# pinterest/rocksplicator

Hardware: NVIDIA H100
Metric: multiget_lookups_per_s (higher is better)
Workload: dtype u8

## Files before the change

rocksplicator_b200/csrc/engine.cu:

```cuda
#include <algorithm>
#include <atomic>
#include <chrono>
#include <cstddef>
#include <cstdio>
#include <cstdlib>
#include <cstring>
#include <deque>
#include <functional>
#include <map>
#include <memory>
#include <mutex>
#include <stdexcept>
#include <string>
#include <thread>
#include <unordered_map>
#include <vector>

#include "../../include/rsp_b200.h"
#include "arena.h"
#include "reader_set.h"
#include "stager.h"
#include "kernels.h"

using namespace rsp;
// ... 163 lines not shown
  mutable bool reserved = false;
};

struct ReadCombiner;
struct ApplyCombiner;
struct Compactor;

struct CudaReaderApi {
  using Stream = cudaStream_t;
  using Event = cudaEvent_t;
  static Event create() {
    cudaEvent_t ev = nullptr;
    CUDA_OK(cudaEventCreateWithFlags(&ev, cudaEventDisableTiming));
    return ev;
  }
  static void record(Event ev, Stream s) { CUDA_OK(cudaEventRecord(ev, s)); }
  static void wait(Stream on, Event ev) { CUDA_OK(cudaStreamWaitEvent(on, ev, 0)); }
  static void destroy(Event ev) { cudaEventDestroy(ev); }
};

struct rsp_engine {
  int device = 0;
  std::mutex comb_mu;
  ReadCombiner* read_comb = nullptr;
  ApplyCombiner* apply_comb = nullptr;
  std::atomic<ReadCombiner*> read_comb_ready{nullptr};
  std::atomic<ApplyCombiner*> apply_comb_ready{nullptr};
  rsp_engine_cfg cfg{};
  std::mutex mu;
  cudaStream_t st = nullptr;
  cudaStream_t cs[3] = {nullptr, nullptr, nullptr};
  cudaEvent_t cs_done[3] = {nullptr, nullptr, nullptr};
  Arena arena;
  ShardDev* d_shards = nullptr;
  ShardFast* d_fast = nullptr;
  std::vector<rsp_shard*> slots;
  std::unordered_map<std::string, rsp_shard*> by_name;
  PinBuf pin_in, pin_out, pin_up, pin_totals;
  DevBuf dev_tick, dev_q, dev_pending, dev_up;
  cudaEvent_t pending_ev = nullptr;
  bool pending_ev_recorded = false;
  cudaStream_t pending_last_stream = nullptr;
  cudaEvent_t up_ev = nullptr;
  bool up_ev_recorded = false;
  std::vector<u32> gid_scratch;
  std::vector<u8> seen_scratch;
  ReaderSet<CudaReaderApi> readers;
  cudaEvent_t mut_ev = nullptr;
  bool mut_recorded = false;
  size_t stage_threads = 1;
  ShardFast* d_fast_runs = nullptr;
  u32* d_mt_filter = nullptr;
  std::atomic<u32> n_multirun{0};
  std::atomic<u32> n_string_append{0};
  struct Compactor* compactor = nullptr;
  u32 mg_parity = 0;
  size_t pending_cap = 0;
  struct {
    bool fast = false, host = false;
    u32 parity = 0;
    size_t n_chunks = 0, chunk = 0;
  } last_mg;
  cudaEvent_t ev0 = nullptr, ev1 = nullptr;
  std::map<std::string, float> last_ms;
  std::atomic<u64> launches{0};
  ScanView* d_snap_views = nullptr;
  std::vector<rsp_snapshot*> snap_slots;
};

static void set_err(rsp_shard* s, const std::string& m) {
  std::lock_guard<std::mutex> g(s->err_mu);
  s->last_error = m;
}

static void wait_readers(rsp_engine* e) { e->readers.wait(e->st); }
static void note_mutation(rsp_engine* e) {
  CUDA_OK(cudaEventRecord(e->mut_ev, e->st));
  e->mut_recorded = true;
}
static void reader_begin(rsp_engine* e, cudaStream_t s) {
  if (s != e->st && e->mut_recorded) CUDA_OK(cudaStreamWaitEvent(s, e->mut_ev, 0));
}
static void reader_end(rsp_engine* e, cudaStream_t s) {
  if (s == e->st) return;
  e->readers.note(s);
}

static void describe_shard(rsp_engine* e, rsp_shard* s, ShardFast* f_out, ShardFast* fr) {
  s->h.n_runs = (u32)s->runs.size();
  for (u32 i = 0; i < RSP_MAX_RUNS; i++) {
    if (i < s->runs.size()) s->h.runs[i] = s->runs[i]->dev();
    else memset(&s->h.runs[i], 0, sizeof(RunDev));
  }
  auto describe = [](const Run& r, ShardFast* f) {
    f->run0_heap = (u64)r.heap; f->run0_hslots = (u64)r.hslots; f->n_buckets = r.n_buckets;
    f->meta = r.ord_bits | (std::min<u32>(r.uniform_units, 255u) << FAST_META_UNITS_SHIFT);
  };
  ShardFast f;
  memset(&f, 0, sizeof(f));
  if (!s->runs.empty()) describe(*s->runs[0], &f);
  memset(fr, 0, sizeof(ShardFast) * RSP_MAX_RUNS);
  for (size_t i = 0; i < s->runs.size() && i < RSP_MAX_RUNS; i++) describe(*s->runs[i], &fr[i]);
  const bool multi_now = s->runs.size() > 1;
  if (multi_now != s->counted_multirun) {
    if (multi_now) e->n_multirun++; else e->n_multirun--;
    s->counted_multirun = multi_now;
// ... 263 lines not shown
      while (at < s->runs.size() && s->runs[at].get() != h.srcs.front().get()) at++;
      bool intact = at + h.n_merged <= s->runs.size();
      for (size_t k = 0; intact && k < h.n_merged; k++) intact = s->runs[at + k].get() == h.srcs[k].get();
      s->merging = false;
      s->bg_first_pinned = nullptr;
      if (!intact) { h.s = nullptr; continue; }
    }
    u64 read_b = 0;
    if (h.has_mem) read_b += (u64)s->h.mt_tail * 16;
    for (auto& r : h.srcs) read_b += r->bytes();
    s->stats.compaction_bytes_read += read_b;
    s->stats.compaction_bytes_written += plan->outs[i]->bytes();
    if (h.has_mem) s->stats.flushes++;
    if (h.has_mem && h.generic_sort) s->stats.flush_comparison_sorts++;
    size_t at = 0;
    if (h.n_merged) {
      while (at < s->runs.size() && s->runs[at].get() != h.srcs.front().get()) at++;
      s->stats.compactions++;
      s->runs.erase(s->runs.begin() + at, s->runs.begin() + at + h.n_merged);
    }
    if (plan->outs[i]->n_ent) s->runs.insert(s->runs.begin() + at, plan->outs[i]);
    if (h.has_mem) {
      s->h.mt_tail = 0;
      s->h.mt_count = 0;
    }
    stage_upload(e, s, mode == COMPACT_MERGE, h.has_mem, &up);
  }
  commit_uploads(e, &up);
  note_mutation(e);
  CUDA_OK(cudaStreamSynchronize(e->st));
  e->last_ms["compact"] = plan->ms;
  e->last_ms["compact_total"] += plan->ms;
  for (u32 i = 0; i < nj; i++) {
    rsp_shard* s = plan->jh[i].s;
    if (s && s->runs.size() >= e->cfg.l0_compaction_trigger && !s->merging) bg_request(e, s);
  }
}

static void compact_shards(rsp_engine* e, const std::vector<rsp_shard*>& shards, bool force_full) {
  CompactPlan plan;
  const CompactMode mode = force_full ? COMPACT_FULL : COMPACT_FLUSH;
  plan_jobs(e, shards, mode, &plan);
  if (plan.jobs.empty()) return;
  wait_readers(e);
  try {
    run_jobs(e, &plan, e->st, e->ev0, e->ev1, &e->pin_totals);
  } catch (...) {
    cudaStreamSynchronize(e->st);
    release_work(e, &plan);
    throw;
  }
  install_jobs(e, &plan, mode);
  release_work(e, &plan);
}

static std::shared_ptr<Run> snapshot_memtable(rsp_engine* e, rsp_shard* s) {
  CompactPlan plan;
  plan_jobs(e, {s}, COMPACT_SNAPSHOT, &plan);
  if (plan.jobs.empty()) return nullptr;
  try {
    run_jobs(e, &plan, e->st, e->ev0, e->ev1, &e->pin_totals);
  } catch (...) {
    cudaStreamSynchronize(e->st);
    release_work(e, &plan);
    throw;
  }
  release_work(e, &plan);
  s->stats.compaction_bytes_read += (u64)s->h.mt_tail * 16;
  return plan.outs[0]->n_ent ? plan.outs[0] : nullptr;
}

static void view_of(const rsp_shard* s, const std::vector<std::shared_ptr<Run>>& pinned, ScanView* v) {
  memset(v, 0, sizeof(*v));
  v->n_runs = (u32)pinned.size();
  v->merge_op = s->opts.merge_op;
  v->merge_delim = s->h.merge_delim;
  for (u32 i = 0; i < v->n_runs; i++) v->runs[i] = pinned[i]->dev();
}

static void pin_view(rsp_engine* e, rsp_shard* s, std::vector<std::shared_ptr<Run>>* pinned, ScanView* v) {
  pinned->clear();
  if (s->h.mt_count) {
    wait_readers(e);
    if (auto snap = snapshot_memtable(e, s)) pinned->push_back(snap);
  }
  pinned->insert(pinned->end(), s->runs.begin(), s->runs.end());
  if (pinned->size() > RSP_MAX_RUNS) {
    pinned->clear();
    compact_shards(e, {s}, false);
    *pinned = s->runs;
  }
  view_of(s, *pinned, v);
}

struct Compactor {
  rsp_engine* e = nullptr;
  std::mutex mu;
  std::condition_variable cv;
  std::vector<rsp_shard*> pending;
  bool stop = false, busy = false;
  cudaStream_t stream = nullptr;
  cudaEvent_t ev0 = nullptr, ev1 = nullptr;
  PinBuf pin_totals;
  std::thread th;
  void loop();
};
// ... 261 lines not shown
    f.chunks = (const ChunkDesc*)(dev + dev_b_base); f.n_chunks = (u32)chunks.size(); f.pad = 0;
    f.chain = (u64*)(dev + dev_b_base + align_up(chunks.size() * sizeof(ChunkDesc), 256));
    f.group_done = (u32*)((u8*)f.chain + chunks.size() * 32);
    if (!chunks.empty())
      CUDA_OK(cudaMemcpyAsync(dev + dev_b_base, chunks.data(), chunks.size() * sizeof(ChunkDesc), cudaMemcpyHostToDevice, e->st));
  }
  if (own_dev) CUDA_OK(cudaStreamSynchronize(e->st));
  return RSP_OK;
}

static void unreserve(const rsp_staged* sg) {
  if (!sg->reserved) return;
  for (size_t g = 0; g < sg->group_shard.size(); g++) {
    rsp_shard* s = sg->group_shard[g];
    s->inflight_units -= std::min<u64>(s->inflight_units, sg->need_units[g]);
    s->inflight_ents -= std::min<u64>(s->inflight_ents, sg->need_ents[g]);
  }
  sg->reserved = false;
}

static inline bool ticks_in_flight(const rsp_shard* s) { return s->inflight_units != 0 || s->inflight_ents != 0; }

static int reserve_for(rsp_engine* e, const rsp_staged* sg) {
  bool did_work = false;
  unreserve(sg);
  auto fits = [](const rsp_shard* s, u64 nu, u64 ne) {
    const u64 tail = (u64)s->h.mt_tail + s->inflight_units, cnt = (u64)s->h.mt_count + s->inflight_ents;
    return tail + nu <= s->h.mt_heap_cap && cnt + ne <= s->h.mt_ent_cap && (cnt + ne) * 2 <= (u64)s->h.mt_slot_mask + 1;
  };
  std::vector<rsp_shard*> to_flush;
  for (size_t g = 0; g < sg->group_shard.size(); g++) {
    rsp_shard* s = sg->group_shard[g];
    if (fits(s, sg->need_units[g], sg->need_ents[g])) continue;
    if (s->inflight_units || s->inflight_ents) return -1;
    if (s->h.mt_count) to_flush.push_back(s);
  }
  if (!to_flush.empty()) { compact_shards(e, to_flush, false); did_work = true; }
  UploadBatch up;
  try {
    for (size_t g = 0; g < sg->group_shard.size(); g++) {
      rsp_shard* s = sg->group_shard[g];
      const u64 nu = sg->need_units[g], ne = sg->need_ents[g];
      if (!fits(s, nu, ne)) {
        alloc_memtable(e, s, nu + nu / 2, ne + ne / 2);
        stage_upload(e, s, false, true, &up);
        did_work = true;
      }
    }
  } catch (...) {
    commit_uploads(e, &up);
    throw;
  }
  commit_uploads(e, &up);
  for (size_t g = 0; g < sg->group_shard.size(); g++) {
    sg->group_shard[g]->inflight_units += sg->need_units[g];
    sg->group_shard[g]->inflight_ents += sg->need_ents[g];
  }
  sg->reserved = true;
  return did_work ? 1 : 0;
}

static void tick_launch(rsp_engine* e, rsp_staged* sg, cudaStream_t st) {
  if (sg->fused) {
    launch_tick_fused(sg->ftick, e->d_shards, e->d_fast, e->d_mt_filter, st);
    CUDA_OK(cudaGetLastError());
    e->launches += 1;
    return;
  }
  launch_decode(sg->tick, st);
  launch_sequence(sg->tick, e->d_shards, e->d_fast, st);
  launch_insert(sg->tick, e->d_shards, e->d_mt_filter, st);
  launch_publish(sg->tick, e->d_shards, st);
  CUDA_OK(cudaGetLastError());
  e->launches += 4;
}

static int tick_results(rsp_engine* e, rsp_staged* sg, cudaStream_t st, int32_t* st_out) {
  u8* pout = (u8*)e->pin_out.get(sg->res_bytes);
  CUDA_OK(cudaMemcpyAsync(pout, sg->tick.gres, sg->res_bytes, cudaMemcpyDeviceToHost, st));
  CUDA_OK(cudaStreamSynchronize(st));
  float ms = 0;
  if (cudaEventElapsedTime(&ms, e->ev0, e->ev1) == cudaSuccess) e->last_ms["apply"] = ms;
  unreserve(sg);
  const size_t ng = sg->group_shard.size();
  const GroupRes* gr = (const GroupRes*)pout;
  const u32* bs = (const u32*)(pout + ng * sizeof(GroupRes));
  int worst = RSP_OK;
  for (size_t g = 0; g < ng; g++) {
    rsp_shard* s = sg->group_shard[g];
    s->h.last_seq = gr[g].last_seq;
    s->h.pub_seq = gr[g].last_seq;
    s->h.mt_tail = gr[g].tail;
    s->h.mt_count = gr[g].count;
    s->h.latch = gr[g].latch;
    s->latch = gr[g].latch;
    s->last_seq.store(gr[g].last_seq, std::memory_order_release);
  }
  bool any_bad = false;
  for (size_t p = 0; p < sg->n; p++) {
    const u32 code = bs[p] >> 8;
    if (st_out) st_out[sg->identity_order ? p : sg->order[p]] = (int32_t)code;
    any_bad |= code != 0;
  }
  if (any_bad) {
    for (size_t g = 0; g < ng; g++) {
      for (u32 p = sg->group_first[g]; p < sg->group_first[g + 1]; p++) {
// ... 205 lines not shown
    size_t n_ops = recs.size();
    if (recs.back().type != kTypeMerge) {
      n_ops--;
      if (recs.back().type == kTypeValue) { has = true; cur = recs.back().v; }
    }
    if (n_ops == 0) {
      if (!has) return RSP_NOT_FOUND;
      *value = cur;
      return RSP_OK;
    }
    const std::string k((const char*)key, klen);
    for (size_t i = n_ops; i-- > 0;) {
      std::string nv;
      if (!host_merge_one(s, k, has, cur, recs[i].v, &nv)) {
        set_err(s, kMsgText[MSG_MERGE_FAILED]);
        return RSP_CORRUPTION;
      }
      cur.swap(nv);
      has = true;
    }
    *value = cur;
    return RSP_OK;
  }
}

static void pending_order(rsp_engine* e, cudaStream_t stream) {
  if (e->pending_ev_recorded && e->pending_last_stream != stream) CUDA_OK(cudaStreamWaitEvent(stream, e->pending_ev, 0));
}
static void pending_mark(rsp_engine* e, cudaStream_t stream) {
  CUDA_OK(cudaEventRecord(e->pending_ev, stream));
  e->pending_ev_recorded = true;
  e->pending_last_stream = stream;
}
static void set_pending(rsp_engine* e, GetArgs& a, size_t n, cudaStream_t stream) {
  pending_order(e, stream);
  if ((n + 8) * 4 > e->pending_cap) {
    if (e->pending_ev_recorded) CUDA_OK(cudaEventSynchronize(e->pending_ev));
    e->pending_cap = std::max<size_t>((n + 8) * 4, e->pending_cap * 2);
    u32* p = (u32*)e->dev_pending.get(e->pending_cap);
    CUDA_OK(cudaMemsetAsync(p, 0, 16, stream));
    e->mg_parity = 0;
  }
  a.n_special = (u32*)e->dev_pending.p;
  a.n_pending = (u32*)e->dev_pending.p + 2;
  a.pending = a.n_pending + 2;
  a.parity = e->mg_parity;
  e->mg_parity ^= 1u;
}

static bool cat_reads(const rsp_engine* e) { return e->n_string_append.load() != 0; }

static void set_engine_args(rsp_engine* e, GetArgs& a) {
  a.shards = e->d_shards; a.fast = e->d_fast; a.max_shards = e->cfg.max_shards;
  a.multirun = e->n_multirun.load() ? 1u : 0u;
}

static inline bool plain_status(int32_t st) { return st == RSP_OK || st == RSP_NOT_FOUND || st == RSP_INCOMPLETE; }

struct LookupRef {
  rsp_shard* s;
  const uint8_t* key;
  size_t klen;
  const ScanView* d_view;
};
template <class Ref>
static void finish_special(rsp_engine* e, size_t n, Ref ref, uint8_t* vals, size_t val_stride, uint32_t* vlen, int32_t* st) {
  for (size_t i = 0; i < n; i++) {
    if (plain_status(st[i])) continue;
    const LookupRef r = ref(i);
    if (st[i] == ST_NEED_HOST_MERGE) {
      std::string v;
      const int rc = host_fold_get(e, r.s, r.key, r.klen, &v, r.d_view);
      st[i] = rc;
      vlen[i] = 0;
      if (rc == RSP_OK) {
        vlen[i] = (u32)v.size();
        if (v.size() > val_stride) st[i] = RSP_INCOMPLETE;
        else memcpy(vals + i * val_stride, v.data(), v.size());
      }
    } else {
      const u32 msg = vlen[i];
      if (r.s) set_err(r.s, msg < MSG_COUNT ? kMsgText[msg] : "error");
      vlen[i] = 0;
    }
  }
}

static int multi_get_locked(rsp_engine* e, size_t n, const uint32_t* shard_ix, const uint8_t* keys, const uint64_t* koff,
                            uint32_t klen_fixed, uint8_t* vals, size_t val_stride, uint32_t* vlen, int32_t* st) {
  if (n == 0) return RSP_OK;
  const size_t key_bytes = klen_fixed ? n * klen_fixed : (size_t)koff[n];
  QLayout L;
  const size_t o_six = L.add(n * 4), o_koff = L.add(klen_fixed ? 0 : (n + 1) * 8), o_keys = L.add(key_bytes + 16);
  const size_t o_vlen = L.add(n * 4), o_st = L.add(n * 4), o_vals = L.add(n * val_stride + 256);
  u8* d = (u8*)e->dev_q.get(L.size);
  const size_t CH = 1u << 18;
  const bool piped = klen_fixed && n >= 2 * CH;
  const size_t n_chunks = piped ? (n + CH - 1) / CH : 1;
  const size_t scratch_u32 = 4 + 2 * n_chunks + n + 16;
  if (e->pending_ev_recorded) {
    CUDA_OK(cudaEventSynchronize(e->pending_ev));
    e->pending_ev_recorded = false;
  }
  if (scratch_u32 * 4 > e->pending_cap) {
    e->pending_cap = std::max(scratch_u32 * 4, e->pending_cap * 2);
    e->dev_pending.get(e->pending_cap);
  }
// ... 1775 lines not shown
```

rocksplicator_b200/csrc/k_read.cu:

```cuda
#include <algorithm>
#include <cstddef>
#include <type_traits>

#include "kernels.h"

namespace rsp {

__device__ __forceinline__ u64 ldcg64(const void* p) { return __ldcg(reinterpret_cast<const unsigned long long*>(p)); }
__device__ __forceinline__ u32 ldcg32(const void* p) { return __ldcg(reinterpret_cast<const u32*>(p)); }

struct CatState {
  u8* out;
  u64 cap;
  u32 len;
  u32 delim;
  u32 gmask;
};
struct NoCat {};

__device__ __noinline__ void cat_put_reversed(u8* out, u64 cap, u64 at, const u8* src, u32 n, u32 delim, u32 gmask) {
  const u32 lanes = __popc(gmask), lane = __popc(gmask & ((1u << (threadIdx.x & 31u)) - 1u));
  for (u32 b = lane; b < n; b += lanes) {
    const u64 p = at + n - 1u - b;
    if (p < cap) out[p] = __ldcg(src + b);
// ... 249 lines not shown
    if ((u64)vlen > a.val_stride) {
      st = 7;
    } else {
      u8* dst = a.vals + (u64)q * a.val_stride;
      if (acc.imm) {
        if (lane == 0) {
#pragma unroll
          for (u32 b = 0; b < 8; b++) dst[b] = (u8)(acc.res_imm >> (8u * b));
        }
      } else if (!acc.in_place(dst)) {
        group_copy_out(dst, acc.res_ptr, vlen, lane, MG_LANES);
      }
    }
  } else if (st != 1 && st != ST_NEED_HOST_MERGE) {
    vlen = msg;
  }
  if (lane == 0) {
    a.st[q] = st;
    a.vlen[q] = vlen;
    if (st != 0 && st != 1 && st != 7 && a.n_special) atomicAdd(a.n_special, 1u);
  }
}

template <bool CAT>
__device__ __noinline__ void lookup_generic(const GetArgs& a, u32 q, u32 lane, u32 gmask, u32 gbase) {
  const u32 six = __ldg(a.shard_ix + q);
  if (six >= a.max_shards || !a.shards[six].live) return answer_invalid(a, q, lane);
  const ShardDev* sd = a.shards + six;
  u32 klen;
  const u8* kp = lookup_key(a, q, klen);
  Acc<CAT> acc;
  acc.init(sd->merge_op, sd->merge_delim);
  acc.set_out(a.vals + (u64)q * a.val_stride, a.val_stride, gmask);
  walk_shard<MG_LANES>(sd, kp, klen, lane, gmask, gbase, acc);
  answer(a, q, lane, acc);
}

template <bool CAT>
__global__ void __launch_bounds__(256) k_multi_get(GetArgs a) {
  const u32 q = (blockIdx.x * blockDim.x + threadIdx.x) / MG_LANES;
  const u32 lane = threadIdx.x & (MG_LANES - 1);
  const u32 gbase = (threadIdx.x & 31u) & ~(MG_LANES - 1u);
  const u32 gmask = ((1u << MG_LANES) - 1u) << gbase;
  if (q >= a.n) return;
  lookup_generic<CAT>(a, q, lane, gmask, gbase);
}

static_assert(offsetof(ShardDev, mt_slot_mask) == 24 && offsetof(ShardDev, pub_seq) == 56, "ShardDev units 0-3");
static_assert(sizeof(ShardFast) == 32, "ShardFast");

constexpr u32 FL = 2;
constexpr u32 MG16_THREADS = 64;
constexpr u32 MG16_MIN_BLOCKS = 20;

__device__ __forceinline__ u64 pol_evict_last() {
  u64 p;
#ifdef RSP_EMUL
  p = 0;
#else
  asm("createpolicy.fractional.L2::evict_last.b64 %0, 1.0;" : "=l"(p));
#endif
  return p;
}
__device__ __forceinline__ uint4 ldg_pol(const uint4* p, u64 pol) {
  uint4 v;
#ifdef RSP_EMUL
  (void)pol;
  v = *p;
#else
  asm("ld.global.nc.L2::cache_hint.v4.u32 {%0,%1,%2,%3}, [%4], %5;"
      : "=r"(v.x), "=r"(v.y), "=r"(v.z), "=r"(v.w) : "l"(p), "l"(pol));
#endif
  return v;
}

template <bool CG>
__device__ __forceinline__ uint4 ld_entry_unit(const uint4* p) {
  if (CG) return __ldcg(p);
  return __ldg(p);
}
template <bool CG, bool BIG>
__device__ __forceinline__ u32 fast_entry(const u8* ent, u32 U, u32 KU, const uint4& kq, u64 snap, u8* dst,
                                          u64 val_stride, u32 lane, u32& vlen_out) {
  const uint4* ep = reinterpret_cast<const uint4*>(ent);
  const uint4 hd = ld_entry_unit<CG>(ep);
  const uint4 ek = ld_entry_unit<CG>(ep + KU);
  const u32 fv = KU + 1;
  uint4 v0 = make_uint4(0, 0, 0, 0), v1 = v0, v2 = v0;
  if (!CG) {
    if (fv + lane < U) v0 = ld_entry_unit<CG>(ep + fv + lane);
    if (fv + lane + 2 < U) v1 = ld_entry_unit<CG>(ep + fv + lane + 2);
    if (fv + lane + 4 < U) v2 = ld_entry_unit<CG>(ep + fv + lane + 4);
  }
  if (ek.x != kq.x || ek.y != kq.y || ek.z != kq.z || ek.w != kq.w || hd.z != 16) return 1;
  const u64 seq = (((u64)hd.y << 32) | hd.x) >> 8;
  const u32 vu = (hd.w + 15u) >> 4;
  if ((hd.x & 0xffu) != kTypeValue || seq > snap || (!CG && fv + vu > U) || (u64)vu * 16u > val_stride || (!BIG && vu > 6)) return 2;
  uint4* out = reinterpret_cast<uint4*>(dst);
  if (CG) {
    for (u32 u = lane; u < vu; u += FL) out[u] = ld_entry_unit<CG>(ep + fv + u);
  } else {
    if (lane < vu) out[lane] = v0;
    if (lane + 2 < vu) out[lane + 2] = v1;
    if (lane + 4 < vu) out[lane + 4] = v2;
    if (BIG)
      for (u32 u = lane + 6; u < vu; u += FL) out[u] = ld_entry_unit<CG>(ep + fv + u);
  }
  vlen_out = hd.w;
  return 0;
}

template <bool BIG>
__device__ __forceinline__ u32 probe_one_run(const uint4& g0, const uint4& g1, const uint4& kq, u64 h, u8* dst, u64 val_stride,
                                             u32 lane, u32 pmask, u32 pbase, u32& vlen) {
  const u8* heap = reinterpret_cast<const u8*>(((u64)g0.y << 32) | g0.x);
  const u32 n_buckets = g1.x, ord_bits = g1.y & 0xffu, U = (g1.y >> FAST_META_UNITS_SHIFT) & 0xffu;
  if (U == 0 || U >= 255) return 2;
  const uint4* hs = reinterpret_cast<const uint4*>(((u64)g0.w << 32) | g0.z);
  u32 bucket = (u32)(((u64)(u32)h * n_buckets) >> 32);
  const u32 tag = (u32)(h >> 32) >> ord_bits;
  u32 m8 = 0, e8 = 1, probe = 0;
  uint4 sv = make_uint4(0, 0, 0, 0);
#pragma unroll 1
  for (;;) {
    if (!m8) {
      if (probe && e8) return 4;
      if (probe == n_buckets) return 4;
      if (probe) bucket = bucket + 1 == n_buckets ? 0 : bucket + 1;
      probe++;
      sv = ldg_pol(hs + (u64)bucket * 2u + lane, pol_evict_last());
      const u32 m = ((sv.x && (sv.x >> ord_bits) == tag) ? 1u : 0u) | ((sv.y && (sv.y >> ord_bits) == tag) ? 2u : 0u) |
                    ((sv.z && (sv.z >> ord_bits) == tag) ? 4u : 0u) | ((sv.w && (sv.w >> ord_bits) == tag) ? 8u : 0u);
      const u32 e = (sv.x == 0 || sv.y == 0 || sv.z == 0 || sv.w == 0) ? 1u : 0u;
      const u32 mine = m | (e << 4);
      const u32 other = __shfl_xor_sync(pmask, mine, 1);
      m8 = lane ? ((other & 15u) | ((mine & 15u) << 4)) : ((mine & 15u) | ((other & 15u) << 4));
      e8 = (mine | other) >> 4;
      if (!m8) continue;
    }
    const u32 p = __ffs(m8) - 1;
    m8 &= m8 - 1;
    const u32 pick = (p & 2u) ? ((p & 1u) ? sv.w : sv.z) : ((p & 1u) ? sv.y : sv.x);
    const u32 val = __shfl_sync(pmask, pick, pbase + (p >> 2));
    const u32 r = fast_entry<false, BIG>(heap + (u64)((val & ((1u << ord_bits) - 1u)) - 1u) * U * 16u, U, 1, kq, ~0ull, dst,
                                         val_stride, lane, vlen);
    if (r == 0) return 0;
    if (r == 2) return 2;
  }
}

template <bool BIG, bool MULTI>
__device__ __forceinline__ void multi_get16(GetArgs a) {
  const u32 q = (blockIdx.x * blockDim.x + threadIdx.x) / FL;
  const u32 lane = threadIdx.x & (FL - 1);
  const u32 pbase = (threadIdx.x & 31u) & ~1u;
  const u32 pmask = 3u << pbase;
  if (q >= a.n) return;
  u32 six = __ldg(a.shard_ix + q);
  const bool bad_shard = six >= a.max_shards;
  if (bad_shard) six = 0;
  const uint4 kq = __ldg(reinterpret_cast<const uint4*>(a.keys) + q);
  const uint4 f0 = __ldg(reinterpret_cast<const uint4*>(a.fast + six));
  const uint4 f1 = __ldg(reinterpret_cast<const uint4*>(a.fast + six) + 1);
  const u32 n_runs = (f1.y >> FAST_META_RUNS_SHIFT) & 0xffu;
  const u64 k0 = ((u64)kq.y << 32) | kq.x, k1 = ((u64)kq.w << 32) | kq.z;
  const u64 h = hash_final(hash_step(hash_step(hash_init(16), k0), k1));
  u8* dst = a.vals + (u64)q * a.val_stride;
  u32 state = 3;
  u32 vlen = 0;
  if ((!MULTI && n_runs > 1) || ((a.val_stride | reinterpret_cast<uintptr_t>(a.vals)) & 15u) || bad_shard || !(f1.y & FAST_META_LIVE)) state = 2;
  bool in_mem = false;
  if (state == 3 && f1.z ) {
    const u32 fb = mt_filter_bit(h);
    const u32 fw = __ldcg(reinterpret_cast<const u32*>(a.fast + (size_t)a.max_shards * (1u + RSP_MAX_RUNS)) + (size_t)six * MT_FILTER_WORDS + (fb >> 5));
    in_mem = (fw >> (fb & 31u)) & 1u;
  }
  if (in_mem) {
    const uint4* dp = reinterpret_cast<const uint4*>(a.shards + six);
    const uint4 d0 = __ldcg(dp), d1 = __ldcg(dp + 1), d3 = __ldcg(dp + 3);
    const u8* heap = reinterpret_cast<const u8*>(((u64)d0.y << 32) | d0.x);
    const u64* sp = reinterpret_cast<const u64*>(((u64)d0.w << 32) | d0.z);
    const u32 mask = d1.z;
    const u64 snap = ((u64)d3.w << 32) | d3.z;
    const u32 tag = hash_tag32(h);
    u32 cand = 0, info = 0;
#pragma unroll
    for (u32 i = 0; i < 4; i++) {
      const u64 sv = ldcg64(sp + (((u32)h + 4u * lane + i) & mask));
      if (sv == 0) { if (!(info >> 8)) info |= (4u * lane + i + 1u) << 8; }
      else if ((u32)(sv >> 32) == tag && !(info >> 8)) { if (!cand) cand = (u32)sv; info++; }
    }
    const u32 o_cand = __shfl_xor_sync(pmask, cand, 1), o_info = __shfl_xor_sync(pmask, info, 1);
    const u32 lo_info = lane ? o_info : info, hi_info = lane ? info : o_info;
    const u32 lo_cand = lane ? o_cand : cand, hi_cand = lane ? cand : o_cand;
    const bool lo_empty = (lo_info >> 8) != 0;
    const u32 n_match = (lo_info & 0xffu) + (lo_empty ? 0u : (hi_info & 0xffu));
    const bool any_empty = lo_empty || (hi_info >> 8) != 0;
    if (n_match == 1) {
      const u32 c = (lo_info & 0xffu) ? lo_cand : hi_cand;
      const u32 r = fast_entry<true, BIG>(heap + (u64)(c - 1u) * 16u, 7, 2, kq, snap, dst, a.val_stride, lane, vlen);
      state = r == 0 ? 0 : 2;
    } else if (n_match > 1 || !any_empty) {
      state = 2;
    }
  }
  if (state == 3) {
    state = 4;
    for (u32 r = 0; r < n_runs; r++) {
      uint4 g0 = f0, g1 = f1;
      if (MULTI && r) {
        const uint4* fr = reinterpret_cast<const uint4*>(a.fast + a.max_shards) + ((u64)six * RSP_MAX_RUNS + r) * 2u;
        g0 = __ldg(fr);
        g1 = __ldg(fr + 1);
      }
      const u32 rs = probe_one_run<BIG>(g0, g1, kq, h, dst, a.val_stride, lane, pmask, pbase, vlen);
      if (rs != 4 || !MULTI) { state = rs; break; }
    }
  }
  if (lane == 0) {
    if (state == 2) {
      a.pending[atomicAdd(a.n_pending + a.parity, 1u)] = q;
    } else {
      a.st[q] = state == 0 ? 0 : 1;
      a.vlen[q] = vlen;
    }
  }
}

template <bool BIG>
__global__ void __launch_bounds__(MG16_THREADS, MG16_MIN_BLOCKS) k_multi_get16(GetArgs a) { multi_get16<BIG, false>(a); }
template <bool BIG>
__global__ void __launch_bounds__(MG16_THREADS, MG16_MIN_BLOCKS) k_multi_get16m(GetArgs a) { multi_get16<BIG, true>(a); }

template <bool CAT>
__global__ void __launch_bounds__(256) k_multi_get_pending(GetArgs a) {
  const u32 lane = threadIdx.x & (MG_LANES - 1);
  const u32 gbase = (threadIdx.x & 31u) & ~(MG_LANES - 1u);
  const u32 gmask = ((1u << MG_LANES) - 1u) << gbase;
  const u32 n = __ldcg(a.n_pending + a.parity);
  const u32 groups = gridDim.x * (blockDim.x / MG_LANES);
  for (u32 i = (blockIdx.x * blockDim.x + threadIdx.x) / MG_LANES; i < n; i += groups)
    lookup_generic<CAT>(a, __ldcg(a.pending + i), lane, gmask, gbase);
}

bool launch_multi_get(const GetArgs& a, bool cat, cudaStream_t s) {
  if (!a.n) return false;
  const u32 per_block = 256 / MG_LANES;
  const u32 grid = (a.n + per_block - 1) / per_block;
  if (a.klen_fixed == 16 && (reinterpret_cast<uintptr_t>(a.keys) & 15u) == 0 && a.pending && a.fast) {
    cudaMemsetAsync(a.n_pending + a.parity, 0, 4, s);
    const u32 g16 = (a.n + MG16_THREADS / FL - 1) / (MG16_THREADS / FL);
    const bool multi = a.multirun != 0;
    if (a.val_stride > 96) {
      if (multi) k_multi_get16m<true><<<g16, MG16_THREADS, 0, s>>>(a); else k_multi_get16<true><<<g16, MG16_THREADS, 0, s>>>(a);
    } else {
      if (multi) k_multi_get16m<false><<<g16, MG16_THREADS, 0, s>>>(a); else k_multi_get16<false><<<g16, MG16_THREADS, 0, s>>>(a);
    }
    if (cat) k_multi_get_pending<true><<<std::min<u32>(grid, DEVICE_SMS), 256, 0, s>>>(a);
    else k_multi_get_pending<false><<<std::min<u32>(grid, DEVICE_SMS), 256, 0, s>>>(a);
    return true;
  }
  if (cat) k_multi_get<true><<<grid, 256, 0, s>>>(a);
  else k_multi_get<false><<<grid, 256, 0, s>>>(a);
  return false;
}

struct DumpVisitor {
  u8* out;
  u64 cap;
  u32 used, n_rec;
  bool done;
  __device__ bool visit(u32 type, const u8* vptr, u32 vlen) {
    const u32 rec = 8u + ((vlen + 3u) & ~3u);
    if ((u64)used + rec <= cap) {
      *reinterpret_cast<u32*>(out + used) = type;
      *reinterpret_cast<u32*>(out + used + 4) = vlen;
      for (u32 b = 0; b < vlen; b++) out[used + 8 + b] = __ldcg(vptr + b);
      n_rec++;
    }
    used += rec;
    if (type != kTypeMerge) done = true;
    return done;
  }
};

__global__ void k_get_versions(VersionsArgs a) {
  const u32 q = blockIdx.x * blockDim.x + threadIdx.x;
  if (q >= a.n) return;
  const u32 lane_in_warp = threadIdx.x & 31u;
  const ShardDev* sd = a.views ? nullptr : a.shards + a.shard_ix[q];
  const u64 o = a.koff[q];
  const u32 klen = (u32)(a.koff[q + 1] - o);
  DumpVisitor v{a.out + (u64)q * a.out_stride, a.out_stride, 0, 0, false};
  if (a.views) {
    const ScanView& vw = a.views[q];
    const u64 h = hash_key(a.keys + o, klen);
    walk_runs<1>(vw.runs, vw.n_runs, a.keys + o, klen, h, 0, 1u << lane_in_warp, lane_in_warp, v);
  } else {
    walk_shard<1>(sd, a.keys + o, klen, 0, 1u << lane_in_warp, lane_in_warp, v);
  }
  a.n_rec[q] = v.n_rec;
  a.need[q] = v.used;
}

void launch_get_versions(const VersionsArgs& a, cudaStream_t s) {
  if (!a.n) return;
  k_get_versions<<<(a.n + 63) / 64, 64, 0, s>>>(a);
}

template <bool CAT>
// ... 414 lines not shown
```

rocksplicator_b200/csrc/kernels.h:

```cpp
#pragma once
#include "format.cuh"

namespace rsp {

constexpr u32 DEVICE_SMS = 132;

struct BatchDesc {
  u32 shard_ix;
  u32 boff;
  u32 len;
  u32 op_base;
  u32 op_cap;
  u32 group;
  u32 pad0, pad1;
};
struct GroupDesc {
  u32 shard_ix;
  u32 first_batch;
  u32 n_batches;
  u32 pad;
};
struct BatchRes {
  u32 status;
  u32 n_ops;
// ... 38 lines not shown
  u32 n_batches;
  u32 index_in_group;
  u32 shard_ix;
  u32 group_chunks;
  u32 pad0, pad1;
};
constexpr u32 FUSED_CHUNK_BATCHES = 128;
constexpr u32 FUSED_STAGE_BYTES = 16384;
struct FusedTick {
  const u8* blob;
  const u64* off;
  const u32* len;
  const u64* ts;
  const GroupDesc* groups;
  u32* bstat;
  GroupRes* gres;
  u32 n_groups;
  u32 n_batches;
  u32 max_group;
  u32 max_len;
  const ChunkDesc* chunks;
  u64* chain;
  u32* group_done;
  u32 n_chunks;
  u32 pad;
};
inline bool fused_small_shape(u32 max_group, u32 max_len) { return max_group <= 64 && max_len <= 4096; }
constexpr u32 FUSED_MAX_BATCH_BYTES = 16384;
void launch_tick_fused(const FusedTick& t, ShardDev* shards, ShardFast* fast, u32* mt_filter, cudaStream_t s);
void launch_decode(const TickDev& t, cudaStream_t s);
void launch_sequence(const TickDev& t, ShardDev* shards, ShardFast* fast, cudaStream_t s);
void launch_insert(const TickDev& t, ShardDev* shards, u32* mt_filter, cudaStream_t s);
void launch_publish(const TickDev& t, ShardDev* shards, cudaStream_t s);

struct GetArgs {
  const ShardDev* shards;
  const ShardFast* fast;
  const u32* shard_ix;
  const u8* keys;
  const u64* koff;
  u32 klen_fixed;
  u8* vals;
  u64 val_stride;
  u32* vlen;
  i32* st;
  u32 n;
  u32* pending;
  u32* n_pending;
  u32 parity;
  u32* n_special;
  u32 max_shards;
  u32 multirun;
};
static_assert(sizeof(GetArgs) == 128, "GetArgs layout is part of k_multi_get16's measured code generation");
bool launch_multi_get(const GetArgs& a, bool cat, cudaStream_t s);

struct ScanView;
struct VersionsArgs {
  const ShardDev* shards;
  const ScanView* views;
  const u32* shard_ix;
  const u8* keys;
  const u64* koff;
  u8* out;
  u64 out_stride;
  u32* n_rec;
  u32* need;
  u32 n;
};
void launch_get_versions(const VersionsArgs& a, cudaStream_t s);

struct ScanView {
  RunDev runs[RSP_MAX_RUNS];
  u32 n_runs;
  u32 merge_op;
  u32 live;
  u32 merge_delim;
};

struct GetAtArgs {
  const ScanView* views;
  const u32* slot;
  const u8* keys;
  const u64* koff;
  u8* vals;
  u64 val_stride;
  u32* vlen;
  i32* st;
  u32* n_special;
  u32 n_views;
  u32 klen_fixed;
  u32 n;
};
void launch_multi_get_at(const GetAtArgs& a, bool cat, cudaStream_t s);
constexpr u32 SCAN_VLEN_HOST_FOLD = 0xffffffffu;
constexpr u32 SCAN_VLEN_MERGE_FAILED = 0xfffffffeu;
constexpr i32 SCAN_ST_TRUNCATED = 1 << 30;
struct ScanArgs {
  const ShardDev* shards;
  const ScanView* views;
  const u32* shard_ix;
  const u8* keys;
  const u64* koff;
  u32 klen_fixed;
  u32 flags;
  u32 max_entries;
// ... 71 lines not shown
```

Measured before the change: 9.175 billion.

## Prefetch memtable filter word and run home buckets early in 16-byte multiget

Adds a host-tracked memtable-live flag and new kernel variants that issue the memtable filter load and the first hash-bucket loads for the first one or two runs early, before the memtable probe finishes, so their latencies overlap instead of forming a dependent chain. Second-run metadata and its prefetched bucket are parked in shared memory to limit register pressure. The memtable path speculatively loads value units bounded by the heap capacity. Launch bounds are relaxed for the new variants, which trades occupancy for more in-flight loads and adds code complexity.

```diff
diff --git a/rocksplicator_b200/csrc/engine.cu b/rocksplicator_b200/csrc/engine.cu
--- a/rocksplicator_b200/csrc/engine.cu
+++ b/rocksplicator_b200/csrc/engine.cu
@@ -239,6 +239,7 @@
   ShardFast* d_fast_runs = nullptr;
   u32* d_mt_filter = nullptr;
   std::atomic<u32> n_multirun{0};
+  std::atomic<u32> mt_live{0};
   std::atomic<u32> n_string_append{0};
   struct Compactor* compactor = nullptr;
   u32 mg_parity = 0;
@@ -608,6 +609,10 @@
   }
   install_jobs(e, &plan, mode);
   release_work(e, &plan);
+  bool mt_live = false;
+  for (const rsp_shard* s : e->slots)
+    if (s && (s->h.mt_count || s->inflight_ents)) { mt_live = true; break; }
+  e->mt_live = mt_live ? 1u : 0u;
 }
 
 static std::shared_ptr<Run> snapshot_memtable(rsp_engine* e, rsp_shard* s) {
@@ -975,6 +980,7 @@
     throw;
   }
   commit_uploads(e, &up);
+  e->mt_live = 1u;
   for (size_t g = 0; g < sg->group_shard.size(); g++) {
     sg->group_shard[g]->inflight_units += sg->need_units[g];
     sg->group_shard[g]->inflight_ents += sg->need_ents[g];
@@ -1286,7 +1292,7 @@
 
 static void set_engine_args(rsp_engine* e, GetArgs& a) {
   a.shards = e->d_shards; a.fast = e->d_fast; a.max_shards = e->cfg.max_shards;
-  a.multirun = e->n_multirun.load() ? 1u : 0u;
+  a.multirun = (e->n_multirun.load() ? GET_MULTIRUN : 0u) | (e->mt_live.load() ? GET_MT_LIVE : 0u);
 }
 
 static inline bool plain_status(int32_t st) { return st == RSP_OK || st == RSP_NOT_FOUND || st == RSP_INCOMPLETE; }
diff --git a/rocksplicator_b200/csrc/k_read.cu b/rocksplicator_b200/csrc/k_read.cu
--- a/rocksplicator_b200/csrc/k_read.cu
+++ b/rocksplicator_b200/csrc/k_read.cu
@@ -325,6 +325,8 @@
 constexpr u32 FL = 2;
 constexpr u32 MG16_THREADS = 64;
 constexpr u32 MG16_MIN_BLOCKS = 20;
+constexpr u32 mg16w_min_blocks(bool big) { return big ? 18 : MG16_MIN_BLOCKS; }
+constexpr u32 mg16m_min_blocks(bool big) { return big ? 14 : 16; }
 
 __device__ __forceinline__ u64 pol_evict_last() {
   u64 p;
@@ -352,7 +354,7 @@
   if (CG) return __ldcg(p);
   return __ldg(p);
 }
-template <bool CG, bool BIG>
+template <bool CG, bool BIG, bool SPEC = !CG>
 __device__ __forceinline__ u32 fast_entry(const u8* ent, u32 U, u32 KU, const uint4& kq, u64 snap, u8* dst,
                                           u64 val_stride, u32 lane, u32& vlen_out) {
   const uint4* ep = reinterpret_cast<const uint4*>(ent);
@@ -360,7 +362,7 @@
   const uint4 ek = ld_entry_unit<CG>(ep + KU);
   const u32 fv = KU + 1;
   uint4 v0 = make_uint4(0, 0, 0, 0), v1 = v0, v2 = v0;
-  if (!CG) {
+  if (SPEC) {
     if (fv + lane < U) v0 = ld_entry_unit<CG>(ep + fv + lane);
     if (fv + lane + 2 < U) v1 = ld_entry_unit<CG>(ep + fv + lane + 2);
     if (fv + lane + 4 < U) v2 = ld_entry_unit<CG>(ep + fv + lane + 4);
@@ -368,9 +370,9 @@
   if (ek.x != kq.x || ek.y != kq.y || ek.z != kq.z || ek.w != kq.w || hd.z != 16) return 1;
   const u64 seq = (((u64)hd.y << 32) | hd.x) >> 8;
   const u32 vu = (hd.w + 15u) >> 4;
-  if ((hd.x & 0xffu) != kTypeValue || seq > snap || (!CG && fv + vu > U) || (u64)vu * 16u > val_stride || (!BIG && vu > 6)) return 2;
+  if ((hd.x & 0xffu) != kTypeValue || seq > snap || (SPEC && fv + vu > U) || (u64)vu * 16u > val_stride || (!BIG && vu > 6)) return 2;
   uint4* out = reinterpret_cast<uint4*>(dst);
-  if (CG) {
+  if (!SPEC) {
     for (u32 u = lane; u < vu; u += FL) out[u] = ld_entry_unit<CG>(ep + fv + u);
   } else {
     if (lane < vu) out[lane] = v0;
@@ -383,9 +385,9 @@
   return 0;
 }
 
-template <bool BIG>
-__device__ __forceinline__ u32 probe_one_run(const uint4& g0, const uint4& g1, const uint4& kq, u64 h, u8* dst, u64 val_stride,
-                                             u32 lane, u32 pmask, u32 pbase, u32& vlen) {
+template <bool BIG, bool PRE = false>
+__device__ __forceinline__ u32 probe_one_run(const uint4& g0, const uint4& g1, uint4 sv, const uint4& kq, u64 h, u8* dst,
+                                             u64 val_stride, u32 lane, u32 pmask, u32 pbase, u32& vlen) {
   const u8* heap = reinterpret_cast<const u8*>(((u64)g0.y << 32) | g0.x);
   const u32 n_buckets = g1.x, ord_bits = g1.y & 0xffu, U = (g1.y >> FAST_META_UNITS_SHIFT) & 0xffu;
   if (U == 0 || U >= 255) return 2;
@@ -393,7 +395,6 @@
   u32 bucket = (u32)(((u64)(u32)h * n_buckets) >> 32);
   const u32 tag = (u32)(h >> 32) >> ord_bits;
   u32 m8 = 0, e8 = 1, probe = 0;
-  uint4 sv = make_uint4(0, 0, 0, 0);
 #pragma unroll 1
   for (;;) {
     if (!m8) {
@@ -401,7 +402,7 @@
       if (probe == n_buckets) return 4;
       if (probe) bucket = bucket + 1 == n_buckets ? 0 : bucket + 1;
       probe++;
-      sv = ldg_pol(hs + (u64)bucket * 2u + lane, pol_evict_last());
+      if (!PRE || probe > 1) sv = ldg_pol(hs + (u64)bucket * 2u + lane, pol_evict_last());
       const u32 m = ((sv.x && (sv.x >> ord_bits) == tag) ? 1u : 0u) | ((sv.y && (sv.y >> ord_bits) == tag) ? 2u : 0u) |
                     ((sv.z && (sv.z >> ord_bits) == tag) ? 4u : 0u) | ((sv.w && (sv.w >> ord_bits) == tag) ? 8u : 0u);
       const u32 e = (sv.x == 0 || sv.y == 0 || sv.z == 0 || sv.w == 0) ? 1u : 0u;
@@ -422,8 +423,19 @@
   }
 }
 
-template <bool BIG, bool MULTI>
+__device__ __forceinline__ uint4 run_home_bucket(const uint4& g0, const uint4& g1, u64 h, u32 lane) {
+  const u32 n_buckets = g1.x, U = (g1.y >> FAST_META_UNITS_SHIFT) & 0xffu;
+  if (U == 0 || U >= 255 || n_buckets == 0) return make_uint4(0, 0, 0, 0);
+  const uint4* hs = reinterpret_cast<const uint4*>(((u64)g0.w << 32) | g0.z);
+  const u32 bucket = (u32)(((u64)(u32)h * n_buckets) >> 32);
+  return ldg_pol(hs + (u64)bucket * 2u + lane, pol_evict_last());
+}
+
+__shared__ uint4 mg16_run1[3 * MG16_THREADS];
+
+template <bool BIG, bool MULTI, bool MT>
 __device__ __forceinline__ void multi_get16(GetArgs a) {
+  constexpr bool PRE = MULTI || MT;
   const u32 q = (blockIdx.x * blockDim.x + threadIdx.x) / FL;
   const u32 lane = threadIdx.x & (FL - 1);
   const u32 pbase = (threadIdx.x & 31u) & ~1u;
@@ -435,18 +447,37 @@
   const uint4 kq = __ldg(reinterpret_cast<const uint4*>(a.keys) + q);
   const uint4 f0 = __ldg(reinterpret_cast<const uint4*>(a.fast + six));
   const uint4 f1 = __ldg(reinterpret_cast<const uint4*>(a.fast + six) + 1);
-  const u32 n_runs = (f1.y >> FAST_META_RUNS_SHIFT) & 0xffu;
   const u64 k0 = ((u64)kq.y << 32) | kq.x, k1 = ((u64)kq.w << 32) | kq.z;
   const u64 h = hash_final(hash_step(hash_step(hash_init(16), k0), k1));
+  const u32 fb = mt_filter_bit(h);
+  const u32* fwp = reinterpret_cast<const u32*>(a.fast + (size_t)a.max_shards * (1u + RSP_MAX_RUNS)) + (size_t)six * MT_FILTER_WORDS + (fb >> 5);
+  u32 fw = 0;
+  if (MT) fw = __ldcg(fwp);
+  uint4 r1a = make_uint4(0, 0, 0, 0), r1b = r1a;
+  if (MULTI) {
+    const uint4* fr = reinterpret_cast<const uint4*>(a.fast + a.max_shards) + ((u64)six * RSP_MAX_RUNS + 1u) * 2u;
+    r1a = __ldg(fr);
+    r1b = __ldg(fr + 1);
+  }
+  const u32 n_runs = (f1.y >> FAST_META_RUNS_SHIFT) & 0xffu;
   u8* dst = a.vals + (u64)q * a.val_stride;
   u32 state = 3;
   u32 vlen = 0;
   if ((!MULTI && n_runs > 1) || ((a.val_stride | reinterpret_cast<uintptr_t>(a.vals)) & 15u) || bad_shard || !(f1.y & FAST_META_LIVE)) state = 2;
   bool in_mem = false;
   if (state == 3 && f1.z ) {
-    const u32 fb = mt_filter_bit(h);
-    const u32 fw = __ldcg(reinterpret_cast<const u32*>(a.fast + (size_t)a.max_shards * (1u + RSP_MAX_RUNS)) + (size_t)six * MT_FILTER_WORDS + (fb >> 5));
+    if (!MT) fw = __ldcg(fwp);
     in_mem = (fw >> (fb & 31u)) & 1u;
+  }
+  uint4 sv0 = make_uint4(0, 0, 0, 0), sv1 = sv0;
+  if (PRE && state == 3) {
+    if (n_runs >= 1) sv0 = run_home_bucket(f0, f1, h, lane);
+    if (MULTI && n_runs >= 2) sv1 = run_home_bucket(r1a, r1b, h, lane);
+  }
+  if (MULTI) {
+    mg16_run1[threadIdx.x] = make_uint4(r1a.x, r1a.y, r1a.z, r1a.w);
+    mg16_run1[MG16_THREADS + threadIdx.x] = make_uint4(r1b.x, r1b.y, 0, 0);
+    mg16_run1[2 * MG16_THREADS + threadIdx.x] = sv1;
   }
   if (in_mem) {
     const uint4* dp = reinterpret_cast<const uint4*>(a.shards + six);
@@ -471,23 +502,32 @@
     const bool any_empty = lo_empty || (hi_info >> 8) != 0;
     if (n_match == 1) {
       const u32 c = (lo_info & 0xffu) ? lo_cand : hi_cand;
-      const u32 r = fast_entry<true, BIG>(heap + (u64)(c - 1u) * 16u, 7, 2, kq, snap, dst, a.val_stride, lane, vlen);
+      u32 r;
+      if (MT) {
+        const u32 off = c - 1u, cap = d1.w;
+        r = fast_entry<true, BIG, true>(heap + (u64)off * 16u, off < cap ? cap - off : 0u, 2, kq, snap, dst, a.val_stride, lane, vlen);
+      } else {
+        r = fast_entry<true, BIG>(heap + (u64)(c - 1u) * 16u, 7, 2, kq, snap, dst, a.val_stride, lane, vlen);
+      }
       state = r == 0 ? 0 : 2;
     } else if (n_match > 1 || !any_empty) {
       state = 2;
     }
   }
   if (state == 3) {
-    state = 4;
-    for (u32 r = 0; r < n_runs; r++) {
-      uint4 g0 = f0, g1 = f1;
-      if (MULTI && r) {
+    state = n_runs ? probe_one_run<BIG, PRE>(f0, f1, sv0, kq, h, dst, a.val_stride, lane, pmask, pbase, vlen) : 4;
+    if (MULTI && state == 4 && n_runs >= 2) {
+      const volatile uint4* st1 = mg16_run1 + threadIdx.x;
+      const uint4 g0 = make_uint4(st1->x, st1->y, st1->z, st1->w);
+      const uint4 g1 = make_uint4(st1[MG16_THREADS].x, st1[MG16_THREADS].y, 0, 0);
+      const uint4 sv = make_uint4(st1[2 * MG16_THREADS].x, st1[2 * MG16_THREADS].y, st1[2 * MG16_THREADS].z, st1[2 * MG16_THREADS].w);
+      state = probe_one_run<BIG, true>(g0, g1, sv, kq, h, dst, a.val_stride, lane, pmask, pbase, vlen);
+      for (u32 r = 2; r < n_runs && state == 4; r++) {
         const uint4* fr = reinterpret_cast<const uint4*>(a.fast + a.max_shards) + ((u64)six * RSP_MAX_RUNS + r) * 2u;
-        g0 = __ldg(fr);
-        g1 = __ldg(fr + 1);
-      }
-      const u32 rs = probe_one_run<BIG>(g0, g1, kq, h, dst, a.val_stride, lane, pmask, pbase, vlen);
-      if (rs != 4 || !MULTI) { state = rs; break; }
+        const uint4 g0 = __ldg(fr), g1 = __ldg(fr + 1);
+        state = probe_one_run<BIG, true>(g0, g1, run_home_bucket(g0, g1, h, lane), kq, h, dst, a.val_stride, lane, pmask,
+                                         pbase, vlen);
+      }
     }
   }
   if (lane == 0) {
@@ -501,9 +541,20 @@
 }
 
 template <bool BIG>
-__global__ void __launch_bounds__(MG16_THREADS, MG16_MIN_BLOCKS) k_multi_get16(GetArgs a) { multi_get16<BIG, false>(a); }
+__global__ void __launch_bounds__(MG16_THREADS, MG16_MIN_BLOCKS) k_multi_get16(GetArgs a) { multi_get16<BIG, false, false>(a); }
 template <bool BIG>
-__global__ void __launch_bounds__(MG16_THREADS, MG16_MIN_BLOCKS) k_multi_get16m(GetArgs a) { multi_get16<BIG, true>(a); }
+__global__ void __launch_bounds__(MG16_THREADS, mg16w_min_blocks(BIG)) k_multi_get16w(GetArgs a) { multi_get16<BIG, false, true>(a); }
+template <bool BIG, bool MT>
+__global__ void __launch_bounds__(MG16_THREADS, mg16m_min_blocks(BIG)) k_multi_get16m(GetArgs a) { multi_get16<BIG, true, MT>(a); }
+
+template <bool BIG>
+static void launch_multi_get16(const GetArgs& a, u32 grid, cudaStream_t s) {
+  const bool multi = a.multirun & GET_MULTIRUN, mt = a.multirun & GET_MT_LIVE;
+  if (multi && mt) k_multi_get16m<BIG, true><<<grid, MG16_THREADS, 0, s>>>(a);
+  else if (multi) k_multi_get16m<BIG, false><<<grid, MG16_THREADS, 0, s>>>(a);
+  else if (mt) k_multi_get16w<BIG><<<grid, MG16_THREADS, 0, s>>>(a);
+  else k_multi_get16<BIG><<<grid, MG16_THREADS, 0, s>>>(a);
+}
 
 template <bool CAT>
 __global__ void __launch_bounds__(256) k_multi_get_pending(GetArgs a) {
@@ -523,12 +574,8 @@
   if (a.klen_fixed == 16 && (reinterpret_cast<uintptr_t>(a.keys) & 15u) == 0 && a.pending && a.fast) {
     cudaMemsetAsync(a.n_pending + a.parity, 0, 4, s);
     const u32 g16 = (a.n + MG16_THREADS / FL - 1) / (MG16_THREADS / FL);
-    const bool multi = a.multirun != 0;
-    if (a.val_stride > 96) {
-      if (multi) k_multi_get16m<true><<<g16, MG16_THREADS, 0, s>>>(a); else k_multi_get16<true><<<g16, MG16_THREADS, 0, s>>>(a);
-    } else {
-      if (multi) k_multi_get16m<false><<<g16, MG16_THREADS, 0, s>>>(a); else k_multi_get16<false><<<g16, MG16_THREADS, 0, s>>>(a);
-    }
+    if (a.val_stride > 96) launch_multi_get16<true>(a, g16, s);
+    else launch_multi_get16<false>(a, g16, s);
     if (cat) k_multi_get_pending<true><<<std::min<u32>(grid, DEVICE_SMS), 256, 0, s>>>(a);
     else k_multi_get_pending<false><<<std::min<u32>(grid, DEVICE_SMS), 256, 0, s>>>(a);
     return true;
diff --git a/rocksplicator_b200/csrc/kernels.h b/rocksplicator_b200/csrc/kernels.h
--- a/rocksplicator_b200/csrc/kernels.h
+++ b/rocksplicator_b200/csrc/kernels.h
@@ -114,6 +114,8 @@
   u32 max_shards;
   u32 multirun;
 };
+constexpr u32 GET_MULTIRUN = 1u;
+constexpr u32 GET_MT_LIVE = 2u;
 static_assert(sizeof(GetArgs) == 128, "GetArgs layout is part of k_multi_get16's measured code generation");
 bool launch_multi_get(const GetArgs& a, bool cat, cudaStream_t s);
 
```

Result: no change. 9.182 billion (median of 6 runs) (+0.1%).
